# PufferAI/PufferLib

Hardware: AMD Instinct MI355X
Metric: env steps/sec end-to-end PPO (rollout+GAE+update), 4096 envs (higher is better)
Workload: dtype f32; 1 GPU; squared d=3 nt=1, 4096 envs/GPU x 128 steps, obs 49->64 f32 rows, MLP 128, 4 minibatches x 4 epochs, bptt 16 (BASELINE configs[1]); global_batch=524288, parallelism=dp1

## Files before the change

pufferlib_amd/csrc/lane_ops.hpp:

```cpp
#pragma once
#include "common.hpp"

namespace pfa {

template <int CTRL>
__device__ __forceinline__ float dpp_f(float x) {
    return __int_as_float(__builtin_amdgcn_update_dpp(0, __float_as_int(x), CTRL, 0xf, 0xf, false));
}
template <int CTRL>
__device__ __forceinline__ int dpp_i(int x) {
    return __builtin_amdgcn_update_dpp(0, x, CTRL, 0xf, 0xf, false);
}

constexpr int kDppXor1 = 0xB1;
constexpr int kDppXor2 = 0x4E;
constexpr int kDppHalfMirror = 0x141;
constexpr int kDppMirror = 0x140;

__device__ __forceinline__ float row16_max(float x) {
    x = fmaxf(x, dpp_f<kDppXor1>(x));
    x = fmaxf(x, dpp_f<kDppXor2>(x));
    x = fmaxf(x, dpp_f<kDppHalfMirror>(x));
    x = fmaxf(x, dpp_f<kDppMirror>(x));
    return x;
}

__device__ __forceinline__ float row16_sum(float x) {
    x = x + dpp_f<kDppXor1>(x);
    x = x + dpp_f<kDppXor2>(x);
    x = x + dpp_f<kDppHalfMirror>(x);
    x = x + dpp_f<kDppMirror>(x);
    return x;
}

__device__ __forceinline__ void row16_argmax(float &best, int &idx) {
#define PFA_ARGMAX_STEP(CTRL)                                   \
    {                                                           \
        const float ob = dpp_f<CTRL>(best);                     \
        const int oi = dpp_i<CTRL>(idx);                        \
        const bool take = (ob > best) | ((ob == best) & (oi < idx));  \
        best = take ? ob : best;                                \
        idx = take ? oi : idx;                                  \
    }
    PFA_ARGMAX_STEP(kDppXor1)
    PFA_ARGMAX_STEP(kDppXor2)
    PFA_ARGMAX_STEP(kDppHalfMirror)
    PFA_ARGMAX_STEP(kDppMirror)
#undef PFA_ARGMAX_STEP
}

}
```

pufferlib_amd/csrc/rollout.hip:

```cpp
#include "common.hpp"
#include "lane_ops.hpp"
#include "mlp_tile.hpp"
#include "philox.hpp"
#include "rollout_tile.hpp"
#include "sampler.hpp"
#include "squared_env.hpp"

namespace pfa {

#ifdef PFA_PROBES
__device__ unsigned long long *g_rtrace = nullptr;
__device__ int g_rtrace_t0 = 0, g_rtrace_steps = 0;
#define PFA_RSTAMP(t, k)                                                                                            \
    do {                                                                                                            \
        if (g_rtrace && blockIdx.x == 0 && (threadIdx.x & 63) == 0 && (t) >= g_rtrace_t0 && (t) < g_rtrace_t0 + g_rtrace_steps) \
            g_rtrace[(((size_t)(threadIdx.x >> 6)) * g_rtrace_steps + ((t) - g_rtrace_t0)) * 8 + (k)] = __builtin_amdgcn_s_memtime(); \
    } while (0)
#else
#define PFA_RSTAMP(t, k) do { } while (0)
#endif

template <int DP, int KS, int MW = kMW>
__global__ void __launch_bounds__(kRollThreads) mlp_forward_sample_kernel(const float *obs, long long rows, MlpView pv,
                                                                         int a, uint32_t heads, const float *noise,
                                                                         uint64_t seed, uint64_t step, long long row_offset,
                                                                         long long *actions, float *logprob, float *entropy,
                                                                         float *value) {
    __shared__ float xs[XTile<DP>::kFloats];
    __shared__ float part[kRollWaves][kPartFloats];
    SliceFrags<DP, KS, MW> w;
    w.load(pv);
    const int le = threadIdx.x >> 4, lo = threadIdx.x & 15;
    const long long tiles = (rows + 15) / 16;
    for (long long tile = blockIdx.x; tile < tiles; tile += gridDim.x) {
        __syncthreads();
        stage_rows<DP>(obs, tile * 16, rows, xs);
        __syncthreads();
        forward_slice<DP, KS, MW>(w, xs, part);
        __syncthreads();
        const long long row = tile * 16 + le;
        const bool ok = row < rows;
        const float q = ok ? noise_lane(noise ? noise + row * a : nullptr, seed, step, (uint64_t)(row_offset + row), lo, a) : 1.0f;
        const LaneSample sm = heads ? sample_lanes_heads(part, le, lo, a, heads, q) : sample_lanes(part, le, lo, a, q);
        if (ok && lo == 0) {
            actions[row] = sm.action;
            logprob[row] = sm.logprob;
            if (entropy) entropy[row] = sm.entropy;
            value[row] = sm.value;
        }
    }
}

template <int DP, int EPW, bool NT1, int KS, int MW = kMW>
__global__ void __launch_bounds__(kRollThreads) rollout_mlp_squared_kernel(SquaredView v, MlpView pv, int a,
                                                                          pfa_experience ex, const float *noise,
                                                                          uint64_t seed, uint64_t step0, long long env_offset,
                                                                          float *live_obs, float *live_rew, uint8_t *live_term,
                                                                          uint8_t *live_trunc, uint8_t *live_mask) {
    constexpr int XS = XTile<DP>::XS;
    __shared__ float xs[XTile<DP>::kFloats];
    __shared__ float part[kRollWaves][kPartFloats];
    __shared__ uint16_t tg[NT1 ? 1 : 16 * kMaxTargets];
    __builtin_amdgcn_s_setprio(3);
    __shared__ RewardTable rtab;
    const int le = threadIdx.x >> 4, lo = threadIdx.x & 15;
    const int e = blockIdx.x * EPW + le;
    const bool env_ok = le < EPW && e < v.n;
    const bool owner = lo == 0 && env_ok;
    const int T = ex.horizon_T;

    SliceFrags<DP, KS, MW> w;
    w.load(pv);

    stage_rows<DP>(live_obs, (long long)blockIdx.x * EPW, v.n, xs, EPW);
    if (NT1) rtab.build(v.d);
    SquaredEnv s;
    Target1 t1;
    float reward = 0.0f;
    bool terminal = false;
    long long filled = 0;
    uint16_t next_cell = 0;
    uint32_t slot = 0;
    const size_t tape_n = (size_t)v.n;
    if (owner) {
        squared_load(v, e, s);
        if (NT1) {
            t1.set(v.tgt[e], v.g);
            filled = v.hdr->rounds_filled;
            slot = s.rounds % (uint32_t)v.tape_rounds;
            next_cell = v.tape[(size_t)slot * tape_n + e];
        } else {
            for (int t = 0; t < v.nt; ++t) tg[le * kMaxTargets + t] = v.tgt[(size_t)t * v.n + e];
        }
        reward = live_rew[e];
        terminal = live_term[e] != 0;
    }
    const bool noise_lane_ok = env_ok && lo < a;
    const float *nz = noise && noise_lane_ok ? noise + (size_t)e * a + lo : nullptr;
    const size_t nz_step = (size_t)v.n * a;
    float q_next = nz ? nz[0] : 1.0f;
    __builtin_amdgcn_s_waitcnt(0x0F70);
    __syncthreads();

    for (int t = 0; t < T; ++t) {
        PFA_RSTAMP(t, 0);
        unstage_rows<DP>(xs, ex.obs + (size_t)t * DP, (long long)blockIdx.x * EPW, v.n, (size_t)T * DP, EPW);
        PFA_RSTAMP(t, 1);
        forward_slice<DP, KS, MW>(w, xs, part);
        PFA_RSTAMP(t, 2);
        lds_barrier();
        PFA_RSTAMP(t, 3);
        const float q = noise ? q_next
                              : (env_ok ? noise_lane(nullptr, seed, step0 + t, (uint64_t)(env_offset + e), lo, a) : 1.0f);
#ifdef PFA_PROBES
        if (q == -12345.678f) PFA_RSTAMP(t, 7);
#endif
        PFA_RSTAMP(t, 4);
        const LaneSample sm = sample_lanes(part, le, lo, a, q);
#ifdef PFA_PROBES
        if (sm.value == 12345.678f) PFA_RSTAMP(t, 7);
#endif
        PFA_RSTAMP(t, 5);
        if (owner) {
            const float stored_reward = reward;
            const bool stored_terminal = terminal;
            float *grid = xs + le * XS;
            if (NT1) {
                if (s.done) {
                    if ((long long)s.rounds >= filled) v.hdr->underrun = 1;
                    squared_reset_nt1(v, s, grid, t1, next_cell, reward, terminal);
                    s.rounds += 1;
                    slot = slot + 1 == (uint32_t)v.tape_rounds ? 0u : slot + 1;
                } else {
                    squared_step_nt1(v, s, grid, t1, rtab, sm.action, reward, terminal);
                }
            } else {
                uint16_t *tc = tg + le * kMaxTargets;
                if (s.done) {
                    if ((long long)s.rounds >= v.hdr->rounds_filled) v.hdr->underrun = 1;
                    const uint16_t *tr = v.tape + (size_t)(s.rounds % (uint32_t)v.tape_rounds) * v.nt * v.n;
                    squared_reset(v, e, s, grid, tr, tc, reward, terminal);
                    s.rounds += 1;
                } else {
                    bool fin;
                    double fr, fs;
                    int fl;
                    squared_step(v, s, grid, tc, sm.action, reward, terminal, fin, fr, fl, fs);
                }
            }
            const size_t row = (size_t)e * T + t;
            ex.rewards[row] = stored_reward;
            ex.dones[row] = stored_terminal ? 1.0f : 0.0f;
            ex.actions[row] = sm.action;
            ex.logprobs[row] = sm.logprob;
            ex.values[row] = sm.value;
            if (NT1) next_cell = v.tape[(size_t)slot * tape_n + e];
        }
        if (nz && t + 1 < T) q_next = nz[(size_t)(t + 1) * nz_step];
        PFA_RSTAMP(t, 6);
        lds_barrier();
        PFA_RSTAMP(t, 7);
    }

    if (owner) {
        squared_store(v, e, s);
        if (NT1) {
            v.tgt[e] = t1.cell;
        } else {
            for (int t = 0; t < v.nt; ++t) v.tgt[(size_t)t * v.n + e] = tg[le * kMaxTargets + t];
        }
        v.fin[e] = 0;
        live_rew[e] = reward;
        live_term[e] = terminal ? 1 : 0;
        live_trunc[e] = 0;
        live_mask[e] = 1;
    }
    unstage_rows<DP>(xs, live_obs, (long long)blockIdx.x * EPW, v.n, (size_t)DP, EPW);
}

__global__ void __launch_bounds__(256) philox_exp_noise_kernel(float *out, long long steps, long long rows, int a, int groups,
                                                               uint64_t seed, uint64_t step0, long long row_offset) {
    const long long total = steps * rows * groups;
    for (long long i = (long long)blockIdx.x * blockDim.x + threadIdx.x; i < total; i += (long long)gridDim.x * blockDim.x) {
        const int j4 = (int)(i % groups);
        const long long tr = i / groups;
        const long long r = tr % rows, t = tr / rows;
        const uint64_t step = step0 + (uint64_t)t, row = (uint64_t)(row_offset + r);
        const u32x4 w = philox4x32_10((uint32_t)row, (uint32_t)j4, (uint32_t)step, (uint32_t)(step >> 32), (uint32_t)seed,
                                      (uint32_t)(seed >> 32));
        float *o = out + (size_t)tr * a + 4 * j4;
        const int left = a - 4 * j4;
        o[0] = -logf(philox_uniform(w.x));
        if (left > 1) o[1] = -logf(philox_uniform(w.y));
        if (left > 2) o[2] = -logf(philox_uniform(w.z));
        if (left > 3) o[3] = -logf(philox_uniform(w.w));
    }
}

struct TilePolicy {
    MlpView pv;
    int obs_dim, obs_stride;
    uint32_t heads;
};

static int check_shape(bool flat, int hidden, int obs_dim, int obs_stride, int a, uint32_t heads) {
    if (flat) {
        PFA_REQUIRE(hidden == kHidden, "mlp: hidden must be %d (got %d)", kHidden, hidden);
    } else {
        PFA_REQUIRE(hidden == 64 || hidden == 128 || hidden == 256 || hidden == 512, "mlp view: hidden %d is not one of 64/128/256/512", hidden);
    }
    PFA_REQUIRE(obs_stride == 16 || obs_stride == 32 || obs_stride == 64 || (flat && (obs_stride == 96 || obs_stride == 128)),
                "mlp: obs_stride must be one of %s (got %d)", flat ? "16/32/64/96/128" : "16/32/64", obs_stride);
    PFA_REQUIRE(obs_dim >= 1 && obs_dim <= obs_stride, "mlp: obs_dim %d out of range", obs_dim);
    PFA_REQUIRE(a >= 1 && a <= 15, "mlp: num_actions must be in 1..15 (got %d)", a);
    PFA_REQUIRE(heads == 0 || (flat && heads_count(heads, a) >= 1), "mlp: head sizes 0x%x do not sum to num_actions %d", heads, a);
    return 0;
}
static int check_dims(const pfa_mlp_dims *d) {
    PFA_REQUIRE(d != nullptr, "mlp: null dims");
    return check_shape(true, d->hidden, d->obs_dim, d->obs_stride, d->num_actions, d->heads);
}
static int check_view(const pfa_mlp_view *p) {
    PFA_REQUIRE(p != nullptr, "mlp view: null");
    PFA_REQUIRE(p->w1 && p->b1 && p->w2 && p->b2 && p->wv && p->bv, "mlp view: null tensor");
    PFA_REQUIRE(p->ldw1 >= p->obs_dim, "mlp view: obs_dim %d / ldw1 %d out of range", p->obs_dim, p->ldw1);
    return check_shape(false, p->hidden, p->obs_dim, p->obs_stride, p->num_actions, 0);
}
static int policy_of_flat(const float *params, const pfa_mlp_dims *d, TilePolicy *out) {
    if (int rc = check_dims(d)) return rc;
    PFA_REQUIRE(params, "mlp: null parameter buffer");
    *out = TilePolicy{mlp_view_of_flat(params, d->obs_stride, d->num_actions), d->obs_dim, d->obs_stride, d->heads};
    return 0;
}
static int policy_of_view(const pfa_mlp_view *p, TilePolicy *out) {
    if (int rc = check_view(p)) return rc;
    *out = TilePolicy{MlpView{p->w1, p->ldw1, p->obs_dim, p->b1, p->w2, p->b2, p->wv, p->bv, p->num_actions, p->hidden}, p->obs_dim,
                      p->obs_stride, 0};
    return 0;
}

template <int DP_, int KS_, int MW_>
struct Tile {
    static constexpr int DP = DP_, KS = KS_, MW = MW_;
};
template <int MW, class Launch>
static void dispatch_stride(const TilePolicy &p, Launch launch) {
    if (p.obs_stride == 64 && p.obs_dim > 48 && p.obs_dim <= 52) return launch(Tile<64, 13, MW>{});
    switch (p.obs_stride) {
        case 16: return launch(Tile<16, 4, MW>{});
        case 32: return launch(Tile<32, 8, MW>{});
        case 64: return launch(Tile<64, 16, MW>{});
    }
    if constexpr (MW == kMW) {
        if (p.obs_stride == 96) return launch(Tile<96, 24, MW>{});
        return launch(Tile<128, 32, MW>{});
    }
}
template <class Launch>
static void dispatch_tile(const TilePolicy &p, Launch launch) {
    switch (p.pv.hidden) {
        case 64: return dispatch_stride<1>(p, launch);
        case 128: return dispatch_stride<2>(p, launch);
        case 256: return dispatch_stride<4>(p, launch);
        default: return dispatch_stride<8>(p, launch);
    }
}

static int launch_forward_sample(const TilePolicy &p, const float *obs, int64_t rows, const float *noise, const pfa_noise_key *key,
                                 int64_t row_offset, int64_t *actions, float *logprob, float *entropy, float *value, pfa_stream_t stream) {
    PFA_REQUIRE(rows >= 0, "mlp.forward: negative rows");
    if (rows == 0) return 0;
    PFA_REQUIRE(obs && actions && logprob && value, "mlp.forward: null buffer");
    PFA_REQUIRE(noise || key, "mlp.forward: need an explicit noise tensor or a Philox key");
    const uint64_t seed = key ? key->seed : 0, step = key ? key->step : 0;
    const int64_t tiles = (rows + 15) / 16;
    const unsigned grid = (unsigned)(tiles < 4096 ? tiles : 4096);
    dispatch_tile(p, [&](auto tile) {
        using T = decltype(tile);
        hipLaunchKernelGGL((mlp_forward_sample_kernel<T::DP, T::KS, T::MW>), dim3(grid), dim3(kRollThreads), 0, (hipStream_t)stream, obs,
                           (long long)rows, p.pv, p.pv.a, p.heads, noise, seed, step, (long long)row_offset, (long long *)actions, logprob,
                           entropy, value);
    });
    PFA_LAUNCH_CHECK();
    return 0;
}

static int launch_rollout_squared(const TilePolicy &p, void *state, const pfa_squared_config *cfg, const pfa_experience *exp,
                                  const float *noise, const pfa_noise_key *key, int64_t env_offset, float *obs, float *rewards,
                                  uint8_t *terminals, uint8_t *truncations, uint8_t *masks, pfa_stream_t stream) {
    PFA_REQUIRE(state && cfg && exp && obs && rewards && terminals && truncations && masks, "rollout: null buffer");
    PFA_REQUIRE(p.heads == 0, "rollout: the fused rollout samples one Discrete head");
    PFA_REQUIRE(cfg->obs_stride == p.obs_stride, "rollout: env obs_stride %d != policy obs_stride %d", cfg->obs_stride, p.obs_stride);
    PFA_REQUIRE(exp->horizon_T >= 1, "rollout: horizon must be >= 1");
    PFA_REQUIRE(exp->obs && exp->actions && exp->logprobs && exp->values && exp->rewards && exp->dones,
                "rollout: null experience buffer");
    PFA_REQUIRE(noise || key, "rollout: need an explicit noise tensor or a Philox key");
    PFA_REQUIRE(cfg->num_targets <= kMaxTargets, "rollout: too many targets");
    SquaredView v = squared_view(state, *cfg);
    const uint64_t seed = key ? key->seed : 0, step = key ? key->step : 0;
    ScopedKernelTimer timer("rollout_mlp_squared", (hipStream_t)stream);
    const unsigned grid = (unsigned)((cfg->num_envs + 15) / 16);
    const bool nt1 = cfg->num_targets == 1;
    dispatch_tile(p, [&](auto tile) {
        using T = decltype(tile);
        auto *kernel = nt1 ? rollout_mlp_squared_kernel<T::DP, 16, true, T::KS, T::MW> : rollout_mlp_squared_kernel<T::DP, 16, false, T::KS, T::MW>;
        hipLaunchKernelGGL(kernel, dim3(grid), dim3(kRollThreads), 0, (hipStream_t)stream, v, p.pv, p.pv.a, *exp, noise, seed, step,
                           (long long)env_offset, obs, rewards, terminals, truncations, masks);
    });
    PFA_LAUNCH_CHECK();
    return 0;
}

}

using namespace pfa;

#ifdef PFA_PROBES
extern "C" int pfa_probe_set_rollout_trace(unsigned long long *buf, int t0, int steps) {
    PFA_CHECK_HIP(hipMemcpyToSymbol(HIP_SYMBOL(g_rtrace), &buf, sizeof(buf)));
    PFA_CHECK_HIP(hipMemcpyToSymbol(HIP_SYMBOL(g_rtrace_t0), &t0, sizeof(t0)));
    PFA_CHECK_HIP(hipMemcpyToSymbol(HIP_SYMBOL(g_rtrace_steps), &steps, sizeof(steps)));
    return 0;
}
#endif

extern "C" int64_t pfa_mlp_param_count(const pfa_mlp_dims *dims) {
    if (check_dims(dims)) return -1;
    return mlp_offsets(dims->obs_stride, dims->num_actions).count;
}

extern "C" int pfa_mlp_forward_sample(const float *obs, int64_t rows, const float *params, const pfa_mlp_dims *dims,
                                      const float *noise, const pfa_noise_key *key, int64_t row_offset, int64_t *actions,
                                      float *logprob, float *entropy, float *value, pfa_stream_t stream) {
    TilePolicy p;
    if (int rc = policy_of_flat(params, dims, &p)) return rc;
    return launch_forward_sample(p, obs, rows, noise, key, row_offset, actions, logprob, entropy, value, stream);
}

extern "C" int pfa_mlp_view_supported(const pfa_mlp_view *p) { return check_view(p) == 0 ? 1 : 0; }

extern "C" int pfa_mlp_view_forward_sample(const float *obs, int64_t rows, const pfa_mlp_view *view, const float *noise,
                                           const pfa_noise_key *key, int64_t row_offset, int64_t *actions, float *logprob,
                                           float *entropy, float *value, pfa_stream_t stream) {
    TilePolicy p;
    if (int rc = policy_of_view(view, &p)) return rc;
    return launch_forward_sample(p, obs, rows, noise, key, row_offset, actions, logprob, entropy, value, stream);
}

extern "C" int pfa_philox_exp_noise(float *out, int64_t steps, int64_t rows, int32_t num_actions, const pfa_noise_key *key,
                                    int64_t row_offset, pfa_stream_t stream) {
    PFA_REQUIRE(steps >= 0 && rows >= 0, "philox noise: negative shape");
    PFA_REQUIRE(num_actions >= 1 && num_actions <= 15, "philox noise: num_actions must be in 1..15 (got %d)", num_actions);
    if (steps == 0 || rows == 0) return 0;
    PFA_REQUIRE(out && key, "philox noise: null buffer");
    const int groups = (num_actions + 3) / 4;
    const long long total = (long long)steps * rows * groups;
    const unsigned grid = (unsigned)((total + 255) / 256 < 65536 ? (total + 255) / 256 : 65536);
    ScopedKernelTimer timer("philox_exp_noise", (hipStream_t)stream);
    hipLaunchKernelGGL(philox_exp_noise_kernel, dim3(grid), dim3(256), 0, (hipStream_t)stream, out, (long long)steps, (long long)rows,
                       (int)num_actions, groups, key->seed, key->step, (long long)row_offset);
    PFA_LAUNCH_CHECK();
    return 0;
}

extern "C" int pfa_rollout_mlp_squared(void *state, const pfa_squared_config *cfg, const float *params,
                                       const pfa_mlp_dims *dims, const pfa_experience *exp, const float *noise,
                                       const pfa_noise_key *key, int64_t env_offset, float *obs, float *rewards,
                                       uint8_t *terminals, uint8_t *truncations, uint8_t *masks, pfa_stream_t stream) {
    TilePolicy p;
    if (int rc = policy_of_flat(params, dims, &p)) return rc;
    return launch_rollout_squared(p, state, cfg, exp, noise, key, env_offset, obs, rewards, terminals, truncations, masks, stream);
}

extern "C" int pfa_rollout_mlp_view_squared(void *state, const pfa_squared_config *cfg, const pfa_mlp_view *view, const pfa_experience *exp,
                                            const float *noise, const pfa_noise_key *key, int64_t env_offset, float *obs, float *rewards,
                                            uint8_t *terminals, uint8_t *truncations, uint8_t *masks, pfa_stream_t stream) {
    TilePolicy p;
    if (int rc = policy_of_view(view, &p)) return rc;
    return launch_rollout_squared(p, state, cfg, exp, noise, key, env_offset, obs, rewards, terminals, truncations, masks, stream);
}
```

pufferlib_amd/csrc/rollout_tile.hpp:

```cpp
#pragma once
#include "common.hpp"
#include "lane_ops.hpp"
#include "mlp_tile.hpp"
#include "philox.hpp"
#include "sampler.hpp"

namespace pfa {

constexpr int kRollThreads = 256;
constexpr int kRollWaves = 4;
constexpr int kMW = kMT / kRollWaves;

struct MlpView {
    const float *w1;
    int ldw1, cols;
    const float *b1;
    const float *w2;
    const float *b2;
    const float *wv;
    const float *bv;
    int a, hidden;
    __device__ __forceinline__ float w2v(int o, int u) const { return o < a ? w2[o * hidden + u] : (o == a ? wv[u] : 0.0f); }
    __device__ __forceinline__ float b2v(int o) const { return o < a ? b2[o] : (o == a ? bv[0] : 0.0f); }
};
inline MlpView mlp_view_of_flat(const float *params, int dp, int a) {
    const MlpOffsets off = mlp_offsets(dp, a);
    return MlpView{params + off.w1, dp, dp, params + off.b1, params + off.w2, params + off.b2, params + off.wv, params + off.bv, a, kHidden};
}

template <int DP, int KS = DP / 4, int MW = kMW>
struct SliceFrags {
    float w1f[MW][KS], b1f[MW][4], w2f[MW][4], bo[4];
    __device__ __forceinline__ void load(const float *params, int a) {
        const MlpOffsets off = mlp_offsets(DP, a);
        const int wv = wave_id(), c = lane_id() & 15, g = lane_id() >> 4;
#pragma unroll
        for (int i = 0; i < MW; ++i) {
            const int m = MW * wv + i;
#pragma unroll
            for (int kk = 0; kk < KS; ++kk) w1f[i][kk] = params[off.w1 + (16 * m + c) * DP + 4 * kk + g];
#pragma unroll
            for (int r = 0; r < 4; ++r) {
                b1f[i][r] = params[off.b1 + 16 * m + 4 * g + r];
                w2f[i][r] = w2v_at(params, off, a, c, 16 * m + 4 * g + r);
            }
        }
#pragma unroll
        for (int r = 0; r < 4; ++r) bo[r] = wv == 0 ? b2v_at(params, off, a, 4 * g + r) : 0.0f;
    }
    __device__ __forceinline__ void load(const MlpView &p) {
        const int wv = wave_id(), c = lane_id() & 15, g = lane_id() >> 4;
#pragma unroll
        for (int i = 0; i < MW; ++i) {
            const int m = MW * wv + i;
#pragma unroll
            for (int kk = 0; kk < KS; ++kk) w1f[i][kk] = 4 * kk + g < p.cols ? p.w1[(size_t)(16 * m + c) * p.ldw1 + 4 * kk + g] : 0.0f;
#pragma unroll
            for (int r = 0; r < 4; ++r) {
                b1f[i][r] = p.b1[16 * m + 4 * g + r];
                w2f[i][r] = p.w2v(c, 16 * m + 4 * g + r);
            }
        }
#pragma unroll
        for (int r = 0; r < 4; ++r) bo[r] = wv == 0 ? p.b2v(4 * g + r) : 0.0f;
    }
};

template <int DP>
__device__ __forceinline__ void stage_rows(const float *src, long long first_row, long long rows, float *xs,
                                           int tile_rows = 16) {
    constexpr int XS = XTile<DP>::XS, V = DP / 4;
    for (int idx = threadIdx.x; idx < 16 * V; idx += kRollThreads) {
        const int r = idx / V, c4 = idx - r * V;
        float4 x = make_float4(0.f, 0.f, 0.f, 0.f);
        if (r < tile_rows && first_row + r < rows) x = *reinterpret_cast<const float4 *>(src + (first_row + r) * DP + 4 * c4);
        float2 *d = reinterpret_cast<float2 *>(xs + r * XS + 4 * c4);
        d[0] = make_float2(x.x, x.y);
        d[1] = make_float2(x.z, x.w);
    }
}

template <int DP>
__device__ __forceinline__ void unstage_rows(const float *xs, float *dst, long long first_row, long long rows, size_t row_stride,
                                             int tile_rows = 16) {
    constexpr int XS = XTile<DP>::XS, V = DP / 4;
    for (int idx = threadIdx.x; idx < tile_rows * V; idx += kRollThreads) {
        const int r = idx / V, c4 = idx - r * V;
        if (first_row + r < rows) {
            const float2 *sp = reinterpret_cast<const float2 *>(xs + r * XS + 4 * c4);
            const float2 lo2 = sp[0], hi2 = sp[1];
            *reinterpret_cast<float4 *>(dst + (size_t)(first_row + r) * row_stride + 4 * c4) = make_float4(lo2.x, lo2.y, hi2.x, hi2.y);
        }
    }
}

template <int DP, int KS = DP / 4, int MW = kMW>
__device__ __forceinline__ void forward_slice(const SliceFrags<DP, KS, MW> &w, const float *xs, float (*part)[kPartFloats]) {
    constexpr int XS = XTile<DP>::XS;
    const int wv = wave_id(), c = lane_id() & 15, g = lane_id() >> 4;
    f32x4 h[MW];
#pragma unroll
    for (int i = 0; i < MW; ++i) h[i] = f32x4{w.b1f[i][0], w.b1f[i][1], w.b1f[i][2], w.b1f[i][3]};
    float bv[KS];
#pragma unroll
    for (int kk = 0; kk < KS; ++kk) bv[kk] = xs[c * XS + 4 * kk + g];
    __builtin_amdgcn_sched_barrier(0);
#pragma unroll
    for (int kk = 0; kk < KS; ++kk) {
#pragma unroll
        for (int i = 0; i < MW; ++i) h[i] = mfma16(w.w1f[i][kk], bv[kk], h[i]);
    }
    f32x4 o0 = f32x4{w.bo[0], w.bo[1], w.bo[2], w.bo[3]}, o1 = f32x4{0.f, 0.f, 0.f, 0.f};
#pragma unroll
    for (int i = 0; i < MW; i += 2) {
#pragma unroll
        for (int r = 0; r < 4; ++r) {
            o0 = mfma16(w.w2f[i][r], fmaxf(h[i][r], 0.0f), o0);
            if constexpr (MW >= 2) o1 = mfma16(w.w2f[i + 1][r], fmaxf(h[i + 1][r], 0.0f), o1);
        }
    }
    const f32x4 po = o0 + o1;
#pragma unroll
    for (int r = 0; r < 4; ++r) part[wv][(4 * g + r) * kPartStride + c] = po[r];
}

__device__ __forceinline__ LaneSample sample_lanes(const float (*part)[kPartFloats], int le, int lo, int a, float q) {
    const int i = lo * kPartStride + le;
    const float mine = (part[0][i] + part[1][i]) + (part[2][i] + part[3][i]);
    return sample_row16(mine, lo, a, q);
}
__device__ __forceinline__ LaneSample sample_lanes_heads(const float (*part)[kPartFloats], int le, int lo, int a, uint32_t heads, float q) {
    const int i = lo * kPartStride + le;
    const float mine = (part[0][i] + part[1][i]) + (part[2][i] + part[3][i]);
    return sample_row16_heads(mine, lo, a, heads, q);
}

}
```

pufferlib_amd/csrc/squared_env.hpp:

```cpp
#pragma once
#include "common.hpp"
#include "mt19937.hpp"

namespace pfa {

constexpr int kMaxTargets = 32;

struct SquaredHeader {
    uint32_t mt[kMtN];
    int32_t mt_idx;
    int32_t underrun;
    unsigned long long words;
    long long rounds_filled;
    double stats[4];
};

struct SquaredView {
    SquaredHeader *hdr;
    int8_t *ax, *ay;
    int32_t *tick;
    uint8_t *done;
    uint32_t *rem;
    uint16_t *tgt;
    uint32_t *rounds;
    double *ep_ret;
    int32_t *ep_len;
    uint8_t *fin;
    double *fin_ret;
    int32_t *fin_len;
    double *fin_score;
    int32_t *acc_cnt;
    double *acc_ret;
    long long *acc_len;
    double *acc_score;
    uint16_t *tape;
    uint32_t *seed_mt;
    int n, d, nt, g, stride, tape_rounds;
};

__host__ __device__ inline size_t sq_carve(size_t &off, size_t bytes) {
    const size_t at = off;
    off = (off + bytes + 255) / 256 * 256;
    return at;
}

__host__ __device__ inline SquaredView squared_view(void *base, const pfa_squared_config &c, size_t *total = nullptr) {
    SquaredView v;
    const size_t N = (size_t)c.num_envs, NT = (size_t)c.num_targets;
    char *p = (char *)base;
    size_t off = 0;
    v.hdr = (SquaredHeader *)(p + sq_carve(off, sizeof(SquaredHeader)));
    v.ax = (int8_t *)(p + sq_carve(off, N));
    v.ay = (int8_t *)(p + sq_carve(off, N));
    v.tick = (int32_t *)(p + sq_carve(off, 4 * N));
    v.done = (uint8_t *)(p + sq_carve(off, N));
    v.rem = (uint32_t *)(p + sq_carve(off, 4 * N));
    v.tgt = (uint16_t *)(p + sq_carve(off, 2 * N * NT));
    v.rounds = (uint32_t *)(p + sq_carve(off, 4 * N));
    v.ep_ret = (double *)(p + sq_carve(off, 8 * N));
    v.ep_len = (int32_t *)(p + sq_carve(off, 4 * N));
    v.fin = (uint8_t *)(p + sq_carve(off, N));
    v.fin_ret = (double *)(p + sq_carve(off, 8 * N));
    v.fin_len = (int32_t *)(p + sq_carve(off, 4 * N));
    v.fin_score = (double *)(p + sq_carve(off, 8 * N));
    v.acc_cnt = (int32_t *)(p + sq_carve(off, 4 * N));
    v.acc_ret = (double *)(p + sq_carve(off, 8 * N));
    v.acc_len = (long long *)(p + sq_carve(off, 8 * N));
    v.acc_score = (double *)(p + sq_carve(off, 8 * N));
    v.tape = (uint16_t *)(p + sq_carve(off, 2 * (size_t)c.tape_rounds * NT * N));
    v.seed_mt = (uint32_t *)(p + sq_carve(off, 4 * (size_t)kMtN * N));
    v.n = c.num_envs;
    v.d = c.distance_to_target;
    v.nt = c.num_targets;
    v.g = 2 * c.distance_to_target + 1;
    v.stride = c.obs_stride;
    v.tape_rounds = c.tape_rounds;
    if (total) *total = off;
    return v;
}

struct SquaredEnv {
    int x, y, tick;
    uint32_t rem;
    uint32_t rounds;
    bool done;
    double ep_ret;
    int ep_len;
    int acc_cnt;
    double acc_ret;
    long long acc_len;
    double acc_score;
};

__device__ __forceinline__ void squared_load(const SquaredView &v, int e, SquaredEnv &s) {
    s.x = v.ax[e];
    s.y = v.ay[e];
    s.tick = v.tick[e];
    s.rem = v.rem[e];
    s.rounds = v.rounds[e];
    s.done = v.done[e] != 0;
    s.ep_ret = v.ep_ret[e];
    s.ep_len = v.ep_len[e];
    s.acc_cnt = v.acc_cnt[e];
    s.acc_ret = v.acc_ret[e];
    s.acc_len = v.acc_len[e];
    s.acc_score = v.acc_score[e];
}

__device__ __forceinline__ void squared_store(const SquaredView &v, int e, const SquaredEnv &s) {
    v.ax[e] = (int8_t)s.x;
    v.ay[e] = (int8_t)s.y;
    v.tick[e] = s.tick;
    v.rem[e] = s.rem;
    v.rounds[e] = s.rounds;
    v.done[e] = s.done ? 1 : 0;
    v.ep_ret[e] = s.ep_ret;
    v.ep_len[e] = s.ep_len;
    v.acc_cnt[e] = s.acc_cnt;
    v.acc_ret[e] = s.acc_ret;
    v.acc_len[e] = s.acc_len;
    v.acc_score[e] = s.acc_score;
}

__device__ __forceinline__ void squared_move(int a, int &dx, int &dy) {
    constexpr uint32_t DX = 0x0u | (0u << 2) | (3u << 4) | (1u << 6) | (1u << 8) | (3u << 10) | (1u << 12) | (3u << 14);
    constexpr uint32_t DY = 0x3u | (1u << 2) | (0u << 4) | (0u << 6) | (3u << 8) | (3u << 10) | (1u << 12) | (1u << 14);
    const int sx = (DX >> (2 * a)) & 3, sy = (DY >> (2 * a)) & 3;
    dx = sx == 3 ? -1 : sx;
    dy = sy == 3 ? -1 : sy;
}

template <typename GridPtr>
__device__ __forceinline__ void squared_reset(const SquaredView &v, int e, SquaredEnv &s, GridPtr grid,
                                              const uint16_t *tape_round , uint16_t *tcells,
                                              float &reward, bool &terminal) {
    const int g = v.g, d = v.d, cells = g * g;
    for (int i = 0; i < cells; ++i) grid[i] = 0.0f;
    grid[d * g + d] = -1.0f;
    s.x = d;
    s.y = d;
    s.tick = 0;
    for (int t = 0; t < v.nt; ++t) {
        const uint16_t c = tape_round[(size_t)t * v.n + e];
        tcells[t] = c;
        grid[c] = 1.0f;
    }
    s.rem = v.nt >= 32 ? 0xffffffffu : ((1u << v.nt) - 1u);
    s.done = false;
    s.ep_ret = 0.0;
    s.ep_len = 0;
    reward = 0.0f;
    terminal = false;
}

template <typename GridPtr>
__device__ __forceinline__ void squared_step(const SquaredView &v, SquaredEnv &s, GridPtr grid, const uint16_t *tcells,
                                             int action, float &reward, bool &terminal, bool &finished,
                                             double &fin_ret, int &fin_len, double &fin_score) {
    const int g = v.g, d = v.d;
    int x = s.x, y = s.y;
    grid[x * g + y] = 0.0f;
    int dx, dy;
    squared_move(action & 7, dx, dy);
    x += dx;
    y += dy;
    int min_dist = 1 << 30;
    int hit = -1;
    for (int t = 0; t < v.nt; ++t) {
        if (!((s.rem >> t) & 1u)) continue;
        const int c = tcells[t];
        const int tx = c / g, ty = c - tx * g;
        const int ddx = x > tx ? x - tx : tx - x, ddy = y > ty ? y - ty : ty - y;
        const int dist = ddx > ddy ? ddx : ddy;
        min_dist = dist < min_dist ? dist : min_dist;
        if (dist == 0 && hit < 0) hit = t;
    }
    const double r = 1.0 - (double)min_dist / (double)d;
    if (hit >= 0) s.rem &= ~(1u << hit);
    const int ox = x > d ? x - d : d - x, oy = y > d ? y - d : d - y;
    if ((ox > oy ? ox : oy) >= d) { x = d; y = d; }
    s.x = x;
    s.y = y;
    grid[x * g + y] = -1.0f;
    s.tick += 1;
    const bool done = s.tick >= v.nt * d;
    s.ep_ret += r;
    s.ep_len += 1;
    finished = done;
    if (done) {
        fin_ret = s.ep_ret;
        fin_len = s.ep_len;
        fin_score = (double)(v.nt - __popc(s.rem)) / (double)v.nt;
        s.acc_cnt += 1;
        s.acc_ret += fin_ret;
        s.acc_len += fin_len;
        s.acc_score += fin_score;
    }
    reward = (float)r;
    terminal = done;
    s.done = done;
}

constexpr int kMaxRewardDist = 32;

struct RewardTable {
    double rd[kMaxRewardDist];
    float rf[kMaxRewardDist];
    __device__ __forceinline__ void build(int d) {
        for (int k = threadIdx.x; k < kMaxRewardDist; k += blockDim.x) {
            const double r = 1.0 - (double)k / (double)d;
            rd[k] = r;
            rf[k] = (float)r;
        }
    }
};

struct Target1 {
    int tx, ty;
    uint16_t cell;
    __device__ __forceinline__ void set(uint16_t c, int g) {
        cell = c;
        tx = c / g;
        ty = c - tx * g;
    }
};

template <typename GridPtr>
__device__ __forceinline__ void squared_reset_nt1(const SquaredView &v, SquaredEnv &s, GridPtr grid, Target1 &tg, uint16_t new_cell,
                                                  float &reward, bool &terminal) {
    const int g = v.g, d = v.d;
    grid[s.x * g + s.y] = 0.0f;
    grid[tg.cell] = 0.0f;
    grid[d * g + d] = -1.0f;
    s.x = d;
    s.y = d;
    s.tick = 0;
    tg.set(new_cell, g);
    grid[new_cell] = 1.0f;
    s.rem = 1u;
    s.done = false;
    s.ep_ret = 0.0;
    s.ep_len = 0;
    reward = 0.0f;
    terminal = false;
}

template <typename GridPtr>
__device__ __forceinline__ void squared_step_nt1(const SquaredView &v, SquaredEnv &s, GridPtr grid, const Target1 &tg,
                                                 const RewardTable &rt, int action, float &reward, bool &terminal) {
    const int g = v.g, d = v.d;
    int x = s.x, y = s.y;
    grid[x * g + y] = 0.0f;
    int dx, dy;
    squared_move(action & 7, dx, dy);
    x += dx;
    y += dy;
    const int ddx = x > tg.tx ? x - tg.tx : tg.tx - x, ddy = y > tg.ty ? y - tg.ty : tg.ty - y;
    const int min_dist = s.rem ? (ddx > ddy ? ddx : ddy) : (1 << 30);
    double r;
    float rf;
    if (min_dist < kMaxRewardDist) {
        r = rt.rd[min_dist];
        rf = rt.rf[min_dist];
    } else {
        r = 1.0 - (double)min_dist / (double)d;
        rf = (float)r;
    }
    if (min_dist == 0) s.rem = 0u;
    const int ox = x > d ? x - d : d - x, oy = y > d ? y - d : d - y;
    if ((ox > oy ? ox : oy) >= d) { x = d; y = d; }
    s.x = x;
    s.y = y;
    grid[x * g + y] = -1.0f;
    s.tick += 1;
    const bool done = s.tick >= d;
    s.ep_ret += r;
    s.ep_len += 1;
    if (done) {
        s.acc_cnt += 1;
        s.acc_ret += s.ep_ret;
        s.acc_len += s.ep_len;
        s.acc_score += s.rem ? 0.0 : 1.0;
    }
    reward = rf;
    terminal = done;
    s.done = done;
}

}
```

Before: 428.6 million env_steps/s.

## Fuse obs unstaging into forward pass and use integer DPP reductions

Moves the per-step copy of staged observations from LDS to the experience buffer inside forward_slice: LDS reads are issued before the first MFMA layer and the global stores after it, so the stores overlap the matmul. Adds a FULL specialization that drops bounds checks when num_envs is a multiple of 16. Replaces the float max and argmax DPP reductions with integer max/min on order-preserving keys, and uses integer-bit ReLU. Also replaces the per-step tape index multiply with an incrementing pointer and uses __mul24 for grid indexing. These are micro-savings in a rollout kernel that is only part of the end-to-end PPO loop, at the cost of extra registers for the held obs values.

Measured after the change: 434.9 million env_steps/s (median of 6 runs). 1.5% higher.

```diff
diff --git a/pufferlib_amd/csrc/lane_ops.hpp b/pufferlib_amd/csrc/lane_ops.hpp
--- a/pufferlib_amd/csrc/lane_ops.hpp
+++ b/pufferlib_amd/csrc/lane_ops.hpp
@@ -7,22 +7,35 @@
 __device__ __forceinline__ float dpp_f(float x) {
     return __int_as_float(__builtin_amdgcn_update_dpp(0, __float_as_int(x), CTRL, 0xf, 0xf, false));
 }
-template <int CTRL>
-__device__ __forceinline__ int dpp_i(int x) {
-    return __builtin_amdgcn_update_dpp(0, x, CTRL, 0xf, 0xf, false);
-}
 
 constexpr int kDppXor1 = 0xB1;
 constexpr int kDppXor2 = 0x4E;
 constexpr int kDppHalfMirror = 0x141;
 constexpr int kDppMirror = 0x140;
 
+template <int CTRL>
+__device__ __forceinline__ int dpp_bc(int x) {
+    return __builtin_amdgcn_update_dpp(0, x, CTRL, 0xf, 0xf, true);
+}
+__device__ __forceinline__ int row16_max_i32(int x) {
+    x = max(x, dpp_bc<kDppXor1>(x));
+    x = max(x, dpp_bc<kDppXor2>(x));
+    x = max(x, dpp_bc<kDppHalfMirror>(x));
+    x = max(x, dpp_bc<kDppMirror>(x));
+    return x;
+}
+__device__ __forceinline__ int row16_min_i32(int x) {
+    x = min(x, dpp_bc<kDppXor1>(x));
+    x = min(x, dpp_bc<kDppXor2>(x));
+    x = min(x, dpp_bc<kDppHalfMirror>(x));
+    x = min(x, dpp_bc<kDppMirror>(x));
+    return x;
+}
+
+__device__ __forceinline__ int float_order_key(int bits) { return bits ^ ((bits >> 31) & 0x7fffffff); }
+
 __device__ __forceinline__ float row16_max(float x) {
-    x = fmaxf(x, dpp_f<kDppXor1>(x));
-    x = fmaxf(x, dpp_f<kDppXor2>(x));
-    x = fmaxf(x, dpp_f<kDppHalfMirror>(x));
-    x = fmaxf(x, dpp_f<kDppMirror>(x));
-    return x;
+    return __int_as_float(float_order_key(row16_max_i32(float_order_key(__float_as_int(x)))));
 }
 
 __device__ __forceinline__ float row16_sum(float x) {
@@ -34,19 +47,10 @@
 }
 
 __device__ __forceinline__ void row16_argmax(float &best, int &idx) {
-#define PFA_ARGMAX_STEP(CTRL)                                   \
-    {                                                           \
-        const float ob = dpp_f<CTRL>(best);                     \
-        const int oi = dpp_i<CTRL>(idx);                        \
-        const bool take = (ob > best) | ((ob == best) & (oi < idx));  \
-        best = take ? ob : best;                                \
-        idx = take ? oi : idx;                                  \
-    }
-    PFA_ARGMAX_STEP(kDppXor1)
-    PFA_ARGMAX_STEP(kDppXor2)
-    PFA_ARGMAX_STEP(kDppHalfMirror)
-    PFA_ARGMAX_STEP(kDppMirror)
-#undef PFA_ARGMAX_STEP
+    const int bits = __float_as_int(best);
+    const int top = row16_max_i32(bits);
+    idx = row16_min_i32(bits == top ? idx : 16);
+    best = __int_as_float(top);
 }
 
 }
diff --git a/pufferlib_amd/csrc/rollout.hip b/pufferlib_amd/csrc/rollout.hip
--- a/pufferlib_amd/csrc/rollout.hip
+++ b/pufferlib_amd/csrc/rollout.hip
@@ -51,13 +51,14 @@
     }
 }
 
-template <int DP, int EPW, bool NT1, int KS, int MW = kMW>
+template <int DP, int EPW, bool NT1, int KS, int MW = kMW, bool FULL = false>
 __global__ void __launch_bounds__(kRollThreads) rollout_mlp_squared_kernel(SquaredView v, MlpView pv, int a,
                                                                           pfa_experience ex, const float *noise,
                                                                           uint64_t seed, uint64_t step0, long long env_offset,
                                                                           float *live_obs, float *live_rew, uint8_t *live_term,
                                                                           uint8_t *live_trunc, uint8_t *live_mask) {
     constexpr int XS = XTile<DP>::XS;
+    static_assert(!FULL || EPW == 16, "FULL: every row of the 16-row tile is an env of this workgroup");
     __shared__ float xs[XTile<DP>::kFloats];
     __shared__ float part[kRollWaves][kPartFloats];
     __shared__ uint16_t tg[NT1 ? 1 : 16 * kMaxTargets];
@@ -65,7 +66,7 @@
     __shared__ RewardTable rtab;
     const int le = threadIdx.x >> 4, lo = threadIdx.x & 15;
     const int e = blockIdx.x * EPW + le;
-    const bool env_ok = le < EPW && e < v.n;
+    const bool env_ok = FULL || (le < EPW && e < v.n);
     const bool owner = lo == 0 && env_ok;
     const int T = ex.horizon_T;
 
@@ -81,6 +82,8 @@
     long long filled = 0;
     uint16_t next_cell = 0;
     uint32_t slot = 0;
+    const uint16_t *const tape_e = v.tape + e;
+    const uint16_t *tape_at = tape_e;
     const size_t tape_n = (size_t)v.n;
     if (owner) {
         squared_load(v, e, s);
@@ -88,7 +91,8 @@
             t1.set(v.tgt[e], v.g);
             filled = v.hdr->rounds_filled;
             slot = s.rounds % (uint32_t)v.tape_rounds;
-            next_cell = v.tape[(size_t)slot * tape_n + e];
+            tape_at = tape_e + (size_t)slot * tape_n;
+            next_cell = *tape_at;
         } else {
             for (int t = 0; t < v.nt; ++t) tg[le * kMaxTargets + t] = v.tgt[(size_t)t * v.n + e];
         }
@@ -104,9 +108,9 @@
 
     for (int t = 0; t < T; ++t) {
         PFA_RSTAMP(t, 0);
-        unstage_rows<DP>(xs, ex.obs + (size_t)t * DP, (long long)blockIdx.x * EPW, v.n, (size_t)T * DP, EPW);
+        forward_slice<DP, KS, MW>(w, xs, part,
+                                  RowStore<DP, FULL>{xs, ex.obs + (size_t)t * DP, (long long)blockIdx.x * EPW, v.n, (size_t)T * DP, EPW});
         PFA_RSTAMP(t, 1);
-        forward_slice<DP, KS, MW>(w, xs, part);
         PFA_RSTAMP(t, 2);
         lds_barrier();
         PFA_RSTAMP(t, 3);
@@ -130,7 +134,9 @@
                     if ((long long)s.rounds >= filled) v.hdr->underrun = 1;
                     squared_reset_nt1(v, s, grid, t1, next_cell, reward, terminal);
                     s.rounds += 1;
-                    slot = slot + 1 == (uint32_t)v.tape_rounds ? 0u : slot + 1;
+                    const bool wrap = slot + 1 == (uint32_t)v.tape_rounds;
+                    slot = wrap ? 0u : slot + 1;
+                    tape_at = wrap ? tape_e : tape_at + tape_n;
                 } else {
                     squared_step_nt1(v, s, grid, t1, rtab, sm.action, reward, terminal);
                 }
@@ -154,7 +160,7 @@
             ex.actions[row] = sm.action;
             ex.logprobs[row] = sm.logprob;
             ex.values[row] = sm.value;
-            if (NT1) next_cell = v.tape[(size_t)slot * tape_n + e];
+            if (NT1) next_cell = *tape_at;
         }
         if (nz && t + 1 < T) q_next = nz[(size_t)(t + 1) * nz_step];
         PFA_RSTAMP(t, 6);
@@ -300,10 +306,11 @@
     const uint64_t seed = key ? key->seed : 0, step = key ? key->step : 0;
     ScopedKernelTimer timer("rollout_mlp_squared", (hipStream_t)stream);
     const unsigned grid = (unsigned)((cfg->num_envs + 15) / 16);
-    const bool nt1 = cfg->num_targets == 1;
+    const bool nt1 = cfg->num_targets == 1, full = cfg->num_envs % 16 == 0;
     dispatch_tile(p, [&](auto tile) {
         using T = decltype(tile);
-        auto *kernel = nt1 ? rollout_mlp_squared_kernel<T::DP, 16, true, T::KS, T::MW> : rollout_mlp_squared_kernel<T::DP, 16, false, T::KS, T::MW>;
+        auto *kernel = nt1 ? (full ? rollout_mlp_squared_kernel<T::DP, 16, true, T::KS, T::MW, true> : rollout_mlp_squared_kernel<T::DP, 16, true, T::KS, T::MW, false>)
+                           : (full ? rollout_mlp_squared_kernel<T::DP, 16, false, T::KS, T::MW, true> : rollout_mlp_squared_kernel<T::DP, 16, false, T::KS, T::MW, false>);
         hipLaunchKernelGGL(kernel, dim3(grid), dim3(kRollThreads), 0, (hipStream_t)stream, v, p.pv, p.pv.a, *exp, noise, seed, step,
                            (long long)env_offset, obs, rewards, terminals, truncations, masks);
     });
diff --git a/pufferlib_amd/csrc/rollout_tile.hpp b/pufferlib_amd/csrc/rollout_tile.hpp
--- a/pufferlib_amd/csrc/rollout_tile.hpp
+++ b/pufferlib_amd/csrc/rollout_tile.hpp
@@ -94,8 +94,50 @@
     }
 }
 
-template <int DP, int KS = DP / 4, int MW = kMW>
-__device__ __forceinline__ void forward_slice(const SliceFrags<DP, KS, MW> &w, const float *xs, float (*part)[kPartFloats]) {
+template <int DP, bool FULL>
+struct RowStore {
+    static constexpr int XS = XTile<DP>::XS, V = DP / 4, kPasses = (16 * V + kRollThreads - 1) / kRollThreads;
+    const float *xs;
+    float *dst;
+    long long first_row, rows;
+    size_t row_stride;
+    int tile_rows;
+    float2 lo2[kPasses], hi2[kPasses];
+    __device__ __forceinline__ bool live(int j) const {
+        if constexpr (FULL) {
+            if (16 * V >= (j + 1) * kRollThreads) return true;
+        }
+        const int idx = threadIdx.x + j * kRollThreads;
+        return idx < (FULL ? 16 : tile_rows) * V && (FULL || first_row + idx / V < rows);
+    }
+    __device__ __forceinline__ void read() {
+#pragma unroll
+        for (int j = 0; j < kPasses; ++j) {
+            const int idx = threadIdx.x + j * kRollThreads, r = idx / V, c4 = idx - r * V;
+            if (live(j)) {
+                const float2 *sp = reinterpret_cast<const float2 *>(xs + r * XS + 4 * c4);
+                lo2[j] = sp[0], hi2[j] = sp[1];
+            }
+        }
+    }
+    __device__ __forceinline__ void store() const {
+#pragma unroll
+        for (int j = 0; j < kPasses; ++j) {
+            const int idx = threadIdx.x + j * kRollThreads, r = idx / V, c4 = idx - r * V;
+            if (live(j))
+                *reinterpret_cast<float4 *>(dst + (size_t)(first_row + r) * row_stride + 4 * c4) =
+                    make_float4(lo2[j].x, lo2[j].y, hi2[j].x, hi2[j].y);
+        }
+    }
+};
+struct NoHook {
+    __device__ __forceinline__ void read() {}
+    __device__ __forceinline__ void store() const {}
+};
+
+template <int DP, int KS = DP / 4, int MW = kMW, class Hook = NoHook>
+__device__ __forceinline__ void forward_slice(const SliceFrags<DP, KS, MW> &w, const float *xs, float (*part)[kPartFloats],
+                                              Hook hook = Hook{}) {
     constexpr int XS = XTile<DP>::XS;
     const int wv = wave_id(), c = lane_id() & 15, g = lane_id() >> 4;
     f32x4 h[MW];
@@ -105,18 +147,22 @@
 #pragma unroll
     for (int kk = 0; kk < KS; ++kk) bv[kk] = xs[c * XS + 4 * kk + g];
     __builtin_amdgcn_sched_barrier(0);
+    hook.read();
+    __builtin_amdgcn_sched_barrier(0);
 #pragma unroll
     for (int kk = 0; kk < KS; ++kk) {
 #pragma unroll
         for (int i = 0; i < MW; ++i) h[i] = mfma16(w.w1f[i][kk], bv[kk], h[i]);
     }
+    hook.store();
+    const auto relu = [](float x) { return __int_as_float(max(__float_as_int(x), 0)); };
     f32x4 o0 = f32x4{w.bo[0], w.bo[1], w.bo[2], w.bo[3]}, o1 = f32x4{0.f, 0.f, 0.f, 0.f};
 #pragma unroll
     for (int i = 0; i < MW; i += 2) {
 #pragma unroll
         for (int r = 0; r < 4; ++r) {
-            o0 = mfma16(w.w2f[i][r], fmaxf(h[i][r], 0.0f), o0);
-            if constexpr (MW >= 2) o1 = mfma16(w.w2f[i + 1][r], fmaxf(h[i + 1][r], 0.0f), o1);
+            o0 = mfma16(w.w2f[i][r], relu(h[i][r]), o0);
+            if constexpr (MW >= 2) o1 = mfma16(w.w2f[i + 1][r], relu(h[i + 1][r]), o1);
         }
     }
     const f32x4 po = o0 + o1;
diff --git a/pufferlib_amd/csrc/squared_env.hpp b/pufferlib_amd/csrc/squared_env.hpp
--- a/pufferlib_amd/csrc/squared_env.hpp
+++ b/pufferlib_amd/csrc/squared_env.hpp
@@ -229,9 +229,9 @@
 __device__ __forceinline__ void squared_reset_nt1(const SquaredView &v, SquaredEnv &s, GridPtr grid, Target1 &tg, uint16_t new_cell,
                                                   float &reward, bool &terminal) {
     const int g = v.g, d = v.d;
-    grid[s.x * g + s.y] = 0.0f;
+    grid[__mul24(s.x, g) + s.y] = 0.0f;
     grid[tg.cell] = 0.0f;
-    grid[d * g + d] = -1.0f;
+    grid[__mul24(d, g) + d] = -1.0f;
     s.x = d;
     s.y = d;
     s.tick = 0;
@@ -250,7 +250,7 @@
                                                  const RewardTable &rt, int action, float &reward, bool &terminal) {
     const int g = v.g, d = v.d;
     int x = s.x, y = s.y;
-    grid[x * g + y] = 0.0f;
+    grid[__mul24(x, g) + y] = 0.0f;
     int dx, dy;
     squared_move(action & 7, dx, dy);
     x += dx;
@@ -271,7 +271,7 @@
     if ((ox > oy ? ox : oy) >= d) { x = d; y = d; }
     s.x = x;
     s.y = y;
-    grid[x * g + y] = -1.0f;
+    grid[__mul24(x, g) + y] = -1.0f;
     s.tick += 1;
     const bool done = s.tick >= d;
     s.ep_ret += r;
```
